# marbl/MHAP

Measured on AMD Instinct MI355X. Metric: overlaps/sec, higher is better.
Workload: dtype int64

## Files before the change

mhap_amd/csrc/kernels.hpp:

```cpp
#pragma once
#include "device_common.hpp"

namespace mhap {

constexpr int HASH_TILE = 1024;
constexpr int WEIGHT_THREADS = 1024;
constexpr int WEIGHT_MAXIT = 24;
constexpr int MH_U = 4;
constexpr int ORD_THREADS = 256;
constexpr int ORD_BINS = 2048;
constexpr int CAND_TQ = 128;
constexpr int CAND_TM = 128;
constexpr int CAND_KS = 32;
constexpr int OVL_THREADS = 128;
#ifndef MH_INV_CT
#define MH_INV_CT 2048
#endif
constexpr int INV_CT = MH_INV_CT;

constexpr int BS_WCLASSES = 6;
constexpr int BS_WMAX = 32;
struct StrandInfo { int32_t valid; int32_t mode; int32_t cnt[BS_WCLASSES + 1]; int32_t pad; };

struct FilterTable {
// ... 22 lines not shown
};

void launch_hash_kmers(hipStream_t st, const ReadDesc* descs, int64_t nstrands, int max_len, const uint8_t* store, int64_t* keys,
                       int32_t* h32, int k, int k2, const uint64_t* luts, int only_mat);
void build_kmer_hash_luts(uint64_t* out);
int weight_grid(int num_cus, int64_t nstrands, int max_len, int k);
bool strand_hashes_from_codes(int length, int k, int k2);
void launch_kmer_weights(hipStream_t st, int num_cus, const ReadDesc* descs, int64_t nstrands, int max_len, const int64_t* keys,
                         uint32_t* wts, uint32_t* perm, uint32_t* slabs, int64_t slab_entries, unsigned long long* counter, int k,
                         const FilterTable& ft, double repeat_weight, StrandInfo* info, bool fused, const uint8_t* store,
                         const uint64_t* luts, const int32_t* order, int32_t* slist);
bool launch_minhash(hipStream_t st, hipStream_t st_weighted, int nblocks, int64_t n_unweighted, int64_t n_weighted, const ReadDesc* descs, int64_t nstrands, const int64_t* keys, const uint32_t* wts,
                    const uint32_t* perm, const StrandInfo* info, const uint8_t* store, const uint64_t* luts, int k, int k2, int H,
                    unsigned long long* counter, int32_t* out_rows, int64_t out_stride, int32_t* out_status, int64_t status_stride,
                    const uint64_t* jump, int jump_na, const int32_t* slist, uint32_t* qbuf, const uint64_t* unjump, const uint64_t* jump_w1, unsigned long long* merge,
                    int max_nk);
size_t minhash_merge_bytes(int nblocks, int H);
void build_xorshift_unjump_tables(int na, int nq, uint64_t* out);
int minhash_wgs_per_cu(int H);
size_t minhash_queue_bytes(int nblocks_total, int H);
int minhash_queue_words(int H);
constexpr int XS_JUMP_LOG2 = 2;
constexpr int XS_JUMP_NQ = BS_WMAX;
#ifndef MH_W1_JUMP_NA
#define MH_W1_JUMP_NA 16
#endif
constexpr int W1_JUMP_NA = MH_W1_JUMP_NA;
inline int w1_jump_tables(int H) { return W1_JUMP_NA + ((H + 1) >> XS_JUMP_LOG2) / W1_JUMP_NA + 1; }
void build_xorshift_jump_tables(int na, int nq, uint64_t* out);
void launch_fix_status(hipStream_t st, int32_t* meta, int64_t nreads);
size_t ordered_lds_bytes(int cap, int code_words, int stage_wide);
void launch_ordered(hipStream_t st, const ReadDesc* descs, int64_t nstrands, int max_len_codes, int max_len, const int32_t* h32,
                    const uint8_t* store, const uint64_t* luts, int k2, int S, int cap, int32_t* out_rows, int64_t out_stride,
                    int32_t* out_meta, int64_t meta_stride, int64_t first = 0, int64_t count = -1);

void launch_candidates(hipStream_t st, const int32_t* minhash, int64_t row_stride, const int32_t* qminhash, int64_t qrow_stride,
                       const int32_t* qlist, int nq, int ne, const int64_t* ids, const int64_t* qids, const int32_t* meta,
                       const int32_t* qmeta, const SearchParams& sp, const long long* rowstart, long long nblocks_tri, Candidate* cand,
                       unsigned long long* cand_count, unsigned long long cand_cap);
constexpr int MHAP_MAX_NUM_HASHES = 8192;
int minhash_waves_per_workgroup(int H);
struct InvIndex {
  uint32_t* ends;
  uint2* items;
  uint32_t nb, shift;
  uint64_t slot_stride;
  uint32_t ne;
  uint32_t grouped;
  uint32_t group_t, class_log;
  uint32_t* lines;
  uint32_t nl_log, line_lb, line_ebits;
  uint32_t tile_entries, tiles;
  uint2* staged;
  uint32_t* tile_counts;
  uint32_t* bin_start;
  uint32_t* bin_long;
};
void launch_query_iota(hipStream_t st, int32_t* qlist, int first, int n);
int index_tile_entries(int ne);
void index_group_params(int64_t entries, InvIndex& ix);
int index_coarse_bins();
bool index_line_params(int64_t entries, uint32_t nb, uint32_t& nl_log, uint32_t& lb, uint32_t& ebits);
size_t index_line_bytes(int H, uint32_t nl_log);
int index_max_buckets_log();
void launch_index_verify(hipStream_t st, const int32_t* minhash, int64_t row_stride, const int32_t* meta, int ne, int H, const InvIndex& ix,
                         unsigned long long* missing);
bool launch_index_build(hipStream_t st, const int32_t* minhash, int64_t row_stride, const int32_t* meta, int ne, int H, const InvIndex& ix);
// ... 33 lines not shown
```

mhap_amd/csrc/mhap_capi.hip:

```cpp
#include <algorithm>
#include <atomic>
#include <cmath>
#include <cstdio>
#include <cstdlib>
#include <chrono>
#include <cstring>
#include <condition_variable>
#include <functional>
#include <mutex>
#include <string>
#include <thread>
#include <vector>

#include "../../include/mhap_hip.h"
static double hp_now() { return std::chrono::duration<double, std::milli>(std::chrono::steady_clock::now().time_since_epoch()).count(); }
#define HPROF(tag) do { if (getenv("MHAP_HOST_PROF")) fprintf(stderr, "[host] %-28s %.3f ms\n", tag, hp_now()); } while (0)
#define DBGSYNC(h, tag) do { if (getenv("MHAP_DEBUG_SYNC")) { fprintf(stderr, "[dbg] %s launched\n", tag); hipError_t _e = hipStreamSynchronize((h)->stream); fprintf(stderr, "[dbg] %s done: %s\n", tag, hipGetErrorString(_e)); } } while (0)
#include "kernels.hpp"
#include "mhap_internal.hpp"
#include "overlap_lane.hpp"

using namespace mhap;

namespace {
// ... 420 lines not shown
    unsigned long long* ctr = h->counters.as<unsigned long long>();
    const ReadDesc* dd = h->descs.as<ReadDesc>();
    HIPCHK(h, hipMemcpyAsync(h->descs.p, h->h_descs, (size_t)nb * sizeof(ReadDesc), hipMemcpyHostToDevice, h->stream));
    HIPCHK(h, hipMemsetAsync(h->counters.p, 0, 256, h->stream));
    const bool fused = k == 16 && k2 == 12;
    if (any_mat) {
      time_begin(h, MHAP_K_HASH);
      launch_hash_kmers(h->stream, dd, nstr, B.max_len, h->store.as<uint8_t>(), h->keys.as<int64_t>(), h->h32.as<int32_t>(), k, k2,
                        h->hash_luts.as<uint64_t>(), 1);
      time_end(h);
      DBGSYNC(h, "hash_kmers");
    }
    HPROF("sketch: descriptors up");
    time_begin(h, MHAP_K_WEIGHT);
    launch_kmer_weights(h->stream, h->num_cus, dd, nstr, B.max_len, h->keys.as<int64_t>(), h->wts.as<uint32_t>(), h->perm.as<uint32_t>(),
                        h->slabs.as<uint32_t>(), slab_entries, ctr + 0, k, h->ft, h->P.repeat_weight, h->info.as<StrandInfo>(), fused,
                        h->store.as<uint8_t>(), h->hash_luts.as<uint64_t>(), d_order, h->slist.as<int32_t>());
    time_end(h);
    DBGSYNC(h, "kmer_weights");
    int per_cu = minhash_wgs_per_cu(H);
    if (const char* e = getenv("MHAP_MINHASH_WGS_PER_CU")) { int v = atoi(e); if (v >= 1 && v <= 8) per_cu = v; }
    int mblocks = h->num_cus * per_cu;
    if (eager_x) mblocks = std::max(per_cu, mblocks - dist_eager_reserve_wgs(h));
    HIPCHK(h, h->mhq.ensure(minhash_queue_bytes(2 * std::max(mblocks, 1), H) * (size_t)(minhash_waves_per_workgroup(H) < 4 ? 4 : 1)));
    HIPCHK(h, h->mhmerge.ensure(minhash_merge_bytes(std::max(mblocks, 1), H)));
    unsigned long long lens[2] = {0, 0};
    HIPCHK(h, hipMemcpyAsync(lens, ctr + 4, 16, hipMemcpyDeviceToHost, h->stream));
    { const int rs = sync_stream(h); if (rs != MHAP_OK) return rs; }
    HPROF("sketch: list lengths back");
    const hipStream_t ost = h->stream;
    auto do_ordered = [&](int64_t first, int64_t count) -> int {
      time_begin(h, MHAP_K_ORDERED, ost);
      launch_ordered(ost, dd, nstr, max_len_codes, B.max_len, h->h32.as<int32_t>(), h->store.as<uint8_t>(), h->hash_luts.as<uint64_t>(), k2, S, h->ord_cap,
                     ord_rows, ord_stride, meta_rows, META_W, first, count);
      time_end(h, ost);
      return MHAP_OK;
    };
    const int ord_first_env = []() { const char* e = getenv("MHAP_ORDERED_FIRST"); return e ? atoi(e) : 0; }();
    const int ord_split_env = []() { const char* e = getenv("MHAP_ORDERED_SPLIT"); const int v = e ? atoi(e) : -1; return v > 100 ? 100 : v; }();
    int64_t batch_read_bases = 0;
    for (int64_t i = 0; i < nb; i++) batch_read_bases += h->h_descs[(size_t)i].length;
    const bool split_pays = batch_read_bases >= 900000000LL && (int64_t)lens[0] >= 4 * (int64_t)lens[1];
    int64_t ord_pre = ord_first_env ? nstr : (nstr * (int64_t)(ord_split_env >= 0 ? ord_split_env : (split_pays ? 55 : 0))) / 100;
    ord_pre &= ~(int64_t)1;
    bool ordered_done = false;
    if (ord_pre > 0 && !eager_x) {
      (void)do_ordered(0, ord_pre);
      ordered_done = ord_pre >= nstr;
      const int nowait = []() { const char* e = getenv("MHAP_ORDERED_NOWAIT"); return e ? atoi(e) : 1; }();
      if (!nowait) {
        HIPCHK(h, hipEventRecord(h->ev_mh_fork, h->stream));
        HIPCHK(h, hipStreamWaitEvent(h->mh_stream, h->ev_mh_fork, 0));
      }
    } else ord_pre = 0;
    if (eager_x) {
      (void)do_ordered(0, nstr);
      ordered_done = true;
      const int rxo = dist_eager_ordered(h, h->stream, ord_rows);
      if (rxo != MHAP_OK) return rxo;
    }
    {
      const int prefill = []() { const char* e = getenv("MHAP_W1_PREFILL"); return e ? atoi(e) : 0; }();
      if (ord_first_env == 2) (void)hipStreamSynchronize(h->stream);
      for (int i = 0; i < prefill; i++) (void)hipMemsetAsync(h->mhq.p, 0, h->mhq.cap, h->stream);
    }
    const size_t t_mh = time_begin(h, MHAP_K_MINHASH);
    const bool mh_forked = launch_minhash(h->stream, h->mh_stream, mblocks, (int64_t)lens[0], (int64_t)lens[1], dd, nstr, h->keys.as<int64_t>(), h->wts.as<uint32_t>(),
// ... 1221 lines not shown
```

mhap_amd/csrc/sketch_kernels.hip:

```cpp
#include <cstdlib>
#include <cstring>

#include "kernels.hpp"
#include <algorithm>
#ifdef MH_ORD_PATHS
#include <cstdio>
#include <string>
#include <vector>
#endif

namespace mhap {

constexpr int HASH_SEG = 4096;
constexpr int HASH_LUT_WORDS = 3 * 256;

void build_kmer_hash_luts(uint64_t* out) {
  const uint64_t c1 = 0x87c37b91114253d5ULL, c2 = 0x4cf5ad432745937fULL;
  const uint32_t d1 = 0xcc9e2d51U, d2 = 0x1b873593U;
  const char* acgt = "ACGT";
  for (int idx = 0; idx < 256; idx++) {
    uint64_t block = 0;
    for (int c = 0; c < 4; c++) block |= (uint64_t)(uint8_t)acgt[(idx >> (2 * c)) & 3] << (16 * c);
    uint64_t k1 = block * c1; k1 = rotl64(k1, 31); k1 *= c2;
    uint64_t k2 = block * c2; k2 = rotl64(k2, 33); k2 *= c1;
    uint32_t a = (uint32_t)block, b = (uint32_t)(block >> 32);
    a *= d1; a = rotl32(a, 15); a *= d2;
    b *= d1; b = rotl32(b, 15); b *= d2;
    out[idx] = k1; out[256 + idx] = k2; out[512 + idx] = (uint64_t)a | ((uint64_t)b << 32);
  }
}

__device__ __forceinline__ uint32_t strand_codes16(const uint8_t* __restrict__ pk, int L, int rcs, int i0) {
  const uint32_t* W = (const uint32_t*)pk;
  const int nd = (((L + 3) >> 2) + 3) >> 2;
  int f0 = rcs ? (L - 16 - i0) : i0;
  if (f0 <= -16 || f0 >= 16 * nd) return 0u;
  int sh = 0;
  if (f0 < 0) { sh = -2 * f0; f0 = 0; }
  const int d = f0 >> 4;
  const uint32_t d0 = W[d], d1 = W[d + 1 < nd ? d + 1 : nd - 1];
  uint32_t x = __builtin_amdgcn_alignbit(d1, d0, (uint32_t)(2 * (f0 & 15))) << sh;
  if (rcs) {
    x = __builtin_bswap32(x);
    x = ((x >> 4) & 0x0f0f0f0fu) | ((x & 0x0f0f0f0fu) << 4);
    x = ((x >> 2) & 0x33333333u) | ((x & 0x33333333u) << 2);
    x = ~x;
  }
  return x;
}

__device__ __forceinline__ uint32_t codes_at(const uint32_t* codes, int p) {
  return __builtin_amdgcn_alignbit(codes[(p >> 4) + 1], codes[p >> 4], (uint32_t)(2 * (p & 15)));
}
__device__ __forceinline__ uint32_t strand_window16(const uint32_t* __restrict__ W, int nd, int L, int rcs, int p) {
  int f0 = rcs ? (L - 16 - p) : p;
  int sh = 0;
  if (f0 < 0) { sh = -2 * f0; f0 = 0; }
  const int i0 = f0 >> 4;
  const uint32_t d0 = W[i0 < nd ? i0 : nd - 1], d1 = W[i0 + 1 < nd ? i0 + 1 : nd - 1];
  uint32_t x = __builtin_amdgcn_alignbit(d1, d0, (uint32_t)(2 * (f0 & 15))) << sh;
  if (rcs) {
    x = __builtin_bswap32(x);
    x = ((x >> 4) & 0x0f0f0f0fu) | ((x & 0x0f0f0f0fu) << 4);
    x = ((x >> 2) & 0x33333333u) | ((x & 0x33333333u) << 2);
    x = ~x;
  }
  return x;
}
__device__ __forceinline__ uint64_t mul5(uint64_t x) {
  uint64_t r;
  asm("v_lshl_add_u64 %0, %1, 2, %1" : "=v"(r) : "v"(x));
  return r;
}
// ... 1765 lines not shown
        float pms = 0.f; (void)hipEventElapsedTime(&pms, pe0, pe1);
        fprintf(stderr, "[minhash w1 prof] launch %.3f ms, %d waves: mean shader clock %.0f MHz (wave-clocks / waves / time)\n", pms, nb * 4,
                pms > 0.f ? tot / ((double)nb * 4.0) / ((double)pms * 1e3) : 0.0);
        fprintf(stderr, "[minhash w1 prof] rows %llu (first-type %llu)  wave-clocks: total %.3g  key load+transpose %.1f%%  first-row slots %.1f%% (%.0f clocks/step)  "
                        "later-row slots %.1f%% (%.0f clocks/step)  drains %.1f%%  candidates/row %.0f\n", hp[4], hp[5], tot, 100.0 * hp[0] / tot, 100.0 * hp[1] / tot,
                hp[5] ? (double)hp[1] / ((double)hp[5] * H) : 0.0, 100.0 * hp[2] / tot, hp[4] > hp[5] ? (double)hp[2] / ((double)(hp[4] - hp[5]) * H) : 0.0,
                100.0 * hp[3] / tot, hp[4] ? (double)hp[6] / (double)hp[4] : 0.0);
      } else
        if (qcap == BS_QCAP) hipLaunchKernelGGL((minhash_w1_kernel<false, true>), dim3(nb), dim3(256), lds1, st, a);
        else hipLaunchKernelGGL((minhash_w1_kernel<false, false>), dim3(nb), dim3(256), lds1, st, a);
      if (a.n_tail > 0)
        hipLaunchKernelGGL(minhash_w1_finish_kernel, dim3((unsigned)((a.n_tail * (long long)H + 255) / 256)), dim3(256), 0, st, a);
      if (witness) snprintf(w1_path, sizeof(w1_path), "w1 n_whole %lld n_tail %lld rmax %d stagger %d", (long long)a.n_whole, (long long)a.n_tail, a.rmax, a.stagger);
    }
    if (witness)
      fprintf(stderr, "[minhash] strands %lld weight-1 %lld weighted %lld nblocks %d: weight-1 launch %s; weighted launch %s\n", (long long)nstrands,
              (long long)n_unweighted, (long long)n_weighted, nblocks, w1_path, nb_w > 0 ? (split ? "split" : "wave") : "none");
    return nb_w > 0;
  }
}


#ifdef MH_ORD_PROF
__device__ unsigned long long g_ord_prof[8];
#define ORD_TICK(k) do { __syncthreads(); if (threadIdx.x == 0) { const unsigned long long t_ = wall_clock64(); atomicAdd(&g_ord_prof[k], t_ - ord_t0); ord_t0 = t_; } } while (0)
#else
#define ORD_TICK(k) do { } while (0)
#endif
#ifdef MH_ORD_PATHS
__device__ uint32_t* g_ord_paths;
#define ORD_PATH_VARS uint32_t ord_att = 0; int ord_lv = 0
#define ORD_PATH_ATT(a) do { ord_att = (uint32_t)(a); } while (0)
#define ORD_PATH_LEVEL(l) do { ord_lv = (l); } while (0)
#define ORD_PATH_HOW(how) do { if (threadIdx.x == 0 && g_ord_paths) g_ord_paths[blockIdx.x] = ord_att | ((uint32_t)(how) << 4) | (stage_wide ? 256u : 0u) | (mat ? 512u : 0u); } while (0)
#define ORD_PATH_NETWORK ORD_PATH_HOW(n > cap ? 4 + ord_lv : 1)
#else
#define ORD_PATH_VARS do { } while (0)
#define ORD_PATH_ATT(a) do { } while (0)
#define ORD_PATH_LEVEL(l) do { } while (0)
#define ORD_PATH_HOW(how) do { } while (0)
#define ORD_PATH_NETWORK do { } while (0)
#endif
__device__ __forceinline__ uint32_t mm3_mul5c(uint32_t h) {
  uint32_t t;
  asm("v_lshl_add_u32 %0, %1, 2, %1" : "=v"(t) : "v"(h));
  return t + 0xe6546b64U;
}
constexpr uint32_t ORD_BUCKET_MAX = 32;
__device__ inline uint64_t okey(int32_t h, int pos) { return ((uint64_t)((uint32_t)h ^ 0x80000000u) << 32) | (uint32_t)pos; }

__global__ __launch_bounds__(ORD_THREADS) void ordered_kernel(const ReadDesc* __restrict__ descs, int64_t nstrands,
                                                              const int32_t* __restrict__ h32, const uint8_t* __restrict__ store,
                                                              const uint64_t* __restrict__ luts, int code_words, int stage_wide, int k2, int S, int cap,
                                                              int32_t* __restrict__ out_rows, int64_t out_stride,
                                                              int32_t* __restrict__ out_meta, int64_t meta_stride, int64_t first) {
  extern __shared__ __attribute__((aligned(16))) char smem[];
  uint32_t* hist = (uint32_t*)smem;
  uint32_t* part = hist + ORD_BINS;
  uint32_t* svars = part + ORD_THREADS;
  uint64_t* buf = (uint64_t*)(svars + 4);
  uint16_t* bstart = (uint16_t*)(buf + cap);
  uint32_t* stage = (uint32_t*)(bstart + ORD_BINS + 2);
  uint16_t* stage16 = (uint16_t*)stage;
  const size_t lut_off = ((size_t)ORD_BINS * 4 + (size_t)ORD_THREADS * 4 + 16 + (size_t)cap * 8 + (size_t)(ORD_BINS + 2) * 2 + (size_t)cap * (stage_wide ? 4 : 2) + 7) & ~(size_t)7;
  uint64_t* lut = (uint64_t*)(smem + lut_off);
  uint32_t* codes = (uint32_t*)(lut + 256);
  uint32_t& s_bin = svars[0]; uint32_t& s_below = svars[1]; uint32_t& s_cnt = svars[2]; uint32_t& s_fill = svars[3];
  const int64_t strand = first + (int64_t)blockIdx.x;
  if (strand >= nstrands) return;
#ifdef MH_ORD_PROF
  unsigned long long ord_t0 = wall_clock64();
#endif
  const ReadDesc rd = descs[strand >> 1];
  const int rcs = (int)(strand & 1);
  const int n = rd.length - k2 + 1;
  int32_t* meta = out_meta + strand * meta_stride;
  if (strand_skipped(rd, rcs) || n < 1) {
    if (threadIdx.x == 0) { meta[0] = 0; meta[1] = n; meta[2] = rd.length; }
    return;
  }
  const bool mat = (rd.flags & MHAP_RD_MAT) != 0;
  const int32_t* hp = h32 + rd.h2_off + (rcs ? rd.h2_stride : 0);
  if (!mat) {
    for (int i = threadIdx.x; i < 256; i += ORD_THREADS) lut[i] = luts[512 + i];
    const int ncw = (rd.length + 15) / 16 + 2;
    for (int wj = threadIdx.x; wj < ncw && wj < code_words; wj += ORD_THREADS) codes[wj] = strand_codes16(store + rd.base_off, rd.length, rcs, 16 * wj);
    __syncthreads();
  }
  ORD_TICK(0);
  auto hget = [&](int i) -> int32_t {
    if (mat) return hp[i];
    const uint32_t cw = codes_at(codes, i);
    uint32_t h = 0;
#pragma unroll
    for (int q = 0; q < 3; q++) {
      const uint64_t kk = lut[(cw >> (8 * q)) & 255u];
      h ^= (uint32_t)kk;         h = rotl32(h, 13); h = mm3_mul5c(h);
      h ^= (uint32_t)(kk >> 32); h = rotl32(h, 13); h = mm3_mul5c(h);
    }
    h ^= 24u;
    return (int32_t)fmix32(h);
  };
  const int K = S < n ? S : n;
  if (threadIdx.x == 0) { meta[0] = K; meta[1] = n; meta[2] = rd.length; }
  if (K <= 0) return;
  ORD_PATH_VARS;

  const double ksig = sqrt((double)K), csig = sqrt((double)cap);
  const double target = fmin((double)K + 7.0 * ksig, (double)cap - 5.0 * csig);
  if (n > cap && target >= (double)K + 3.0 * ksig) {
    const double quant = target / (double)n;
    const uint32_t cut_u = quant >= 1.0 ? 0xFFFFFFFFu : (uint32_t)(quant * 4294967296.0);
    const uint32_t cutbin = cut_u >> 21;
    for (uint32_t j = threadIdx.x; j < ORD_BINS; j += ORD_THREADS) hist[j] = 0;
    if (threadIdx.x == 0) { s_fill = 0; s_cnt = 0; }
    __syncthreads();
    const int lane = threadIdx.x & 63;
    for (int ib = 0; ib < n; ib += 8 * ORD_THREADS) {
      const int p0 = ib + 32 * (int)(threadIdx.x >> 2) + (int)(threadIdx.x & 3);
      int32_t hv[8];
      if (mat) {
#pragma unroll
        for (int u = 0; u < 8; u++) { const int i = p0 + 4 * u; hv[u] = i < n ? hp[i] : 0; }
      } else if (p0 < n) {
        const int d = p0 >> 4;
        const uint32_t sh = (uint32_t)(2 * (p0 & 15));
        const uint32_t w0 = codes[d], w1 = codes[d + 1], w2 = codes[d + 2], w3 = codes[d + 3];
        const uint32_t a[3] = {__builtin_amdgcn_alignbit(w1, w0, sh), __builtin_amdgcn_alignbit(w2, w1, sh), __builtin_amdgcn_alignbit(w3, w2, sh)};
        uint64_t g[10];
#pragma unroll
        for (int j = 0; j < 10; j++) g[j] = lut[(a[j >> 2] >> (8 * (j & 3))) & 255u];
#pragma unroll
        for (int u = 0; u < 8; u++) {
          uint32_t h = 0;
#pragma unroll
          for (int q = 0; q < 3; q++) {
            const uint64_t kk = g[u + q];
            h ^= (uint32_t)kk;         h = rotl32(h, 13); h = mm3_mul5c(h);
            h ^= (uint32_t)(kk >> 32); h = rotl32(h, 13); h = mm3_mul5c(h);
          }
          h ^= 24u;
          hv[u] = (int32_t)fmix32(h);
        }
      } else {
#pragma unroll
        for (int u = 0; u < 8; u++) hv[u] = 0;
      }
      unsigned long long bal[8];
      uint32_t total = 0;
#pragma unroll
      for (int u = 0; u < 8; u++) {
        bal[u] = __ballot(p0 + 4 * u < n && ((uint32_t)hv[u] ^ 0x80000000u) < cut_u);
        total += (uint32_t)__popcll(bal[u]);
      }
      if (total) {
        uint32_t base = 0;
        if (lane == 0) base = atomicAdd(&s_fill, total);
        base = (uint32_t)__builtin_amdgcn_readfirstlane((int)base);
#pragma unroll
        for (int u = 0; u < 8; u++) {
          if ((bal[u] >> lane) & 1ULL) {
            const uint32_t idx = base + __builtin_amdgcn_mbcnt_hi((uint32_t)(bal[u] >> 32), __builtin_amdgcn_mbcnt_lo((uint32_t)bal[u], 0u));
            if (idx < (uint32_t)cap) { if (stage_wide) stage[idx] = (uint32_t)(p0 + 4 * u); else stage16[idx] = (uint16_t)(p0 + 4 * u); }
            atomicAdd(&hist[((uint32_t)hv[u] ^ 0x80000000u) >> 21], 1u);
          }
          base += (uint32_t)__popcll(bal[u]);
        }
      }
    }
    __syncthreads();
    ORD_TICK(1);
    const uint32_t m = s_fill;
    bool ok = m >= (uint32_t)K && m <= (uint32_t)cap;
    ORD_PATH_ATT(m < (uint32_t)K ? 2 : m > (uint32_t)cap ? 3 : 1);
    if (ok) {
      const int per = ORD_BINS / ORD_THREADS;
      uint32_t loc = 0, mx = 0;
      for (int j = 0; j < per; j++) { const uint32_t c = hist[threadIdx.x * per + j]; loc += c; mx = c > mx ? c : mx; }
      uint32_t incl = loc;
#pragma unroll
      for (int off = 1; off < 64; off <<= 1) { const uint32_t v = __shfl_up(incl, off); if (lane >= off) incl += v; }
      if (lane == 63) part[threadIdx.x >> 6] = incl;
      if (mx > ORD_BUCKET_MAX) atomicMax(&s_cnt, mx);
      __syncthreads();
      for (unsigned w = 0; w < (threadIdx.x >> 6); w++) incl += part[w];
      uint32_t run = incl - loc;
      for (int j = 0; j < per; j++) { const uint32_t b = threadIdx.x * per + j; bstart[b] = (uint16_t)run; run += hist[b]; }
      ok = s_cnt == 0;
      __syncthreads();
      if (!ok) ORD_PATH_ATT(4);
    }
    ORD_TICK(2);
    if (ok) {
      for (uint32_t b = threadIdx.x; b <= cutbin; b += ORD_THREADS) hist[b] = 0;
      __syncthreads();
      for (uint32_t t0 = threadIdx.x; t0 < m; t0 += 4 * ORD_THREADS) {
        int ii[4]; uint64_t key[4]; uint32_t slot[4];
#pragma unroll
        for (int u = 0; u < 4; u++) { const uint32_t t = t0 + (uint32_t)u * ORD_THREADS; ii[u] = t < m ? (stage_wide ? (int)stage[t] : (int)stage16[t]) : 0; }
#pragma unroll
        for (int u = 0; u < 4; u++) key[u] = okey(hget(ii[u]), ii[u]);
#pragma unroll
        for (int u = 0; u < 4; u++) { const uint32_t b = (uint32_t)(key[u] >> 53); slot[u] = t0 + (uint32_t)u * ORD_THREADS < m ? (uint32_t)bstart[b] + atomicAdd(&hist[b], 1u) : 0xFFFFFFFFu; }
#pragma unroll
        for (int u = 0; u < 4; u++) if (slot[u] != 0xFFFFFFFFu) buf[slot[u]] = key[u];
      }
      __syncthreads();
      ORD_TICK(3);
      int32_t* orow = out_rows + strand * out_stride;
      for (uint32_t t0 = threadIdx.x; t0 < m; t0 += 2 * ORD_THREADS) {
        uint64_t key[2]; uint32_t s0[2], c[2], rank[2] = {0u, 0u};
#pragma unroll
        for (int u = 0; u < 2; u++) {
          const uint32_t t = t0 + (uint32_t)u * ORD_THREADS;
          key[u] = buf[t < m ? t : t0];
          const uint32_t b = (uint32_t)(key[u] >> 53);
          s0[u] = bstart[b]; c[u] = t < m ? hist[b] : 0u;
        }
        const uint32_t cmax = c[0] > c[1] ? c[0] : c[1];
        for (uint32_t q = 0; q < cmax; q += 4) {
          uint64_t o[2][4];
#pragma unroll
          for (int u = 0; u < 2; u++)
#pragma unroll
            for (int x = 0; x < 4; x++) o[u][x] = buf[s0[u] + q + (uint32_t)x < (uint32_t)cap ? s0[u] + q + (uint32_t)x : s0[u]];
#pragma unroll
          for (int u = 0; u < 2; u++)
#pragma unroll
            for (int x = 0; x < 4; x++) rank[u] += (q + (uint32_t)x < c[u] && o[u][x] < key[u]) ? 1u : 0u;
        }
#pragma unroll
        for (int u = 0; u < 2; u++) {
          const uint32_t j = s0[u] + rank[u];
          if (t0 + (uint32_t)u * ORD_THREADS < m && j < (uint32_t)K) { orow[2 * j] = (int32_t)((uint32_t)(key[u] >> 32) ^ 0x80000000u); orow[2 * j + 1] = (int32_t)(uint32_t)key[u]; }
        }
      }
      ORD_TICK(5);
#ifdef MH_ORD_PROF
      if (threadIdx.x == 0) atomicAdd(&g_ord_prof[7], 1ULL);
#endif
      ORD_PATH_HOW(2);
      return;
    }
    __syncthreads();
  }

  uint64_t bound = ~0ULL;
  bool buckets = false;
  uint32_t bk_bin = 0, bk_total = 0;
  if (threadIdx.x == 0) s_fill = 0;
  if (n > cap) {
    const int shifts[6] = {53, 42, 32, 21, 10, 0};
    const int widths[6] = {11, 11, 10, 11, 11, 10};
    uint64_t prefix = 0;
    uint64_t prefmask = 0;
    uint32_t below = 0;
    for (int lv = 0; lv < 6; lv++) {
      const int sh = shifts[lv];
      const uint32_t nb = 1u << widths[lv];
      for (uint32_t j = threadIdx.x; j < ORD_BINS; j += ORD_THREADS) hist[j] = 0;
      __syncthreads();
      for (int i0 = threadIdx.x; i0 < n; i0 += 8 * ORD_THREADS) {
        int32_t hv[8];
#pragma unroll
        for (int u = 0; u < 8; u++) { const int i = i0 + u * ORD_THREADS; hv[u] = i < n ? hget(i) : 0; }
#pragma unroll
        for (int u = 0; u < 8; u++) {
// ... 86 lines not shown
    ORD_PATH_HOW(3);
    return;
  }
  ORD_PATH_NETWORK;
  __syncthreads();
  for (int i = threadIdx.x; i < n; i += ORD_THREADS) {
    const uint64_t key = okey(hget(i), i);
    if (key <= bound) { uint32_t slot = atomicAdd(&s_fill, 1u); if (slot < (uint32_t)cap) buf[slot] = key; }
  }
  __syncthreads();
  const uint32_t m = s_fill < (uint32_t)cap ? s_fill : (uint32_t)cap;
  uint32_t np2 = 1;
  while (np2 < m) np2 <<= 1;
  for (uint32_t j = m + threadIdx.x; j < np2; j += ORD_THREADS) buf[j] = ~0ULL;
  __syncthreads();
  for (uint32_t size = 2; size <= np2; size <<= 1) {
    for (uint32_t stride = size >> 1; stride > 0; stride >>= 1) {
      for (uint32_t t = threadIdx.x; t < (np2 >> 1); t += ORD_THREADS) {
        const uint32_t lo = 2 * t - (t & (stride - 1));
        const uint32_t hi = lo + stride;
        const bool up = ((lo & size) == 0);
        const uint64_t a = buf[lo], b = buf[hi];
        if ((a > b) == up) { buf[lo] = b; buf[hi] = a; }
      }
      __syncthreads();
    }
  }
  int32_t* orow = out_rows + strand * out_stride;
  for (int j = threadIdx.x; j < K; j += ORD_THREADS) {
    const uint64_t key = buf[j];
    orow[2 * j] = (int32_t)((uint32_t)(key >> 32) ^ 0x80000000u);
    orow[2 * j + 1] = (int32_t)(uint32_t)key;
  }
}

#ifndef MH_ORD_PAD
#define MH_ORD_PAD 0
#endif
size_t ordered_lds_bytes(int cap, int code_words, int stage_wide) {
  return (size_t)ORD_BINS * 4 + (size_t)ORD_THREADS * 4 + 16 + (size_t)cap * 8 + (size_t)(ORD_BINS + 2) * 2 + (size_t)cap * (stage_wide ? 4 : 2) +
         (code_words > 0 ? (size_t)256 * 8 + (size_t)code_words * 4 : 0) + 8 + MH_ORD_PAD;
}

__global__ void fix_status_kernel(int32_t* __restrict__ meta, int64_t nreads) {
  const int64_t i = (int64_t)blockIdx.x * blockDim.x + threadIdx.x;
  if (i >= nreads) return;
  const int32_t fs = meta[(2 * i) * META_W + 3];
  if (fs != 0 && meta[(2 * i + 1) * META_W + 3] == 0) meta[(2 * i + 1) * META_W + 3] = fs;
}

void launch_fix_status(hipStream_t st, int32_t* meta, int64_t nreads) {
  if (nreads <= 0) return;
  hipLaunchKernelGGL(fix_status_kernel, dim3((unsigned)((nreads + 255) / 256)), dim3(256), 0, st, meta, nreads);
}

void launch_ordered(hipStream_t st, const ReadDesc* descs, int64_t nstrands, int max_len_codes, int max_len, const int32_t* h32,
                    const uint8_t* store, const uint64_t* luts, int k2, int S, int cap, int32_t* out_rows, int64_t out_stride,
                    int32_t* out_meta, int64_t meta_stride, int64_t first, int64_t count) {
  if (count < 0 || first + count > nstrands) count = nstrands - first;
  if (nstrands <= 0 || count <= 0) return;
  const int code_words = max_len_codes > 0 ? (max_len_codes + 15) / 16 + 4 : 0;
  const int stage_wide = max_len - k2 + 1 > 65535 ? 1 : 0;
#ifdef MH_ORD_PATHS
  uint32_t* d_paths = nullptr;
  if (hipMalloc(&d_paths, (size_t)count * sizeof(uint32_t)) != hipSuccess) d_paths = nullptr;
  if (d_paths) (void)hipMemsetAsync(d_paths, 0, (size_t)count * sizeof(uint32_t), st);
  (void)hipStreamSynchronize(st);
  (void)hipMemcpyToSymbol(HIP_SYMBOL(g_ord_paths), &d_paths, sizeof(d_paths));
#endif
  hipLaunchKernelGGL(ordered_kernel, dim3((unsigned)count), dim3(ORD_THREADS), ordered_lds_bytes(cap, code_words, stage_wide), st, descs, nstrands, h32,
                     store, luts, code_words, stage_wide, k2, S, cap, out_rows, out_stride, out_meta, meta_stride, first);
#ifdef MH_ORD_PROF
  (void)hipStreamSynchronize(st);
  unsigned long long hp[8];
  (void)hipMemcpyFromSymbol(hp, HIP_SYMBOL(g_ord_prof), sizeof(hp));
  fprintf(stderr, "[ordered prof] cap %d lds %zu strands(one-pass) %llu  100MHz ticks/strand: stage %.1f pass1 %.1f scan %.1f fill %.1f isort %.1f out %.1f\n", cap,
          ordered_lds_bytes(cap, code_words, stage_wide), hp[7], (double)hp[0] / hp[7], (double)hp[1] / hp[7], (double)hp[2] / hp[7], (double)hp[3] / hp[7],
          (double)hp[4] / hp[7], (double)hp[5] / hp[7]);
  unsigned long long z[8] = {0, 0, 0, 0, 0, 0, 0, 0};
  (void)hipMemcpyToSymbol(HIP_SYMBOL(g_ord_prof), z, sizeof(z));
#endif
#ifdef MH_ORD_PATHS
  {
    std::vector<uint32_t> h_paths((size_t)count, 0u);
    if (d_paths) (void)hipMemcpyAsync(h_paths.data(), d_paths, (size_t)count * sizeof(uint32_t), hipMemcpyDeviceToHost, st);
    (void)hipStreamSynchronize(st);
    if (d_paths) (void)hipFree(d_paths);
    std::string line;
    line.reserve((size_t)count * 4 + 96);
    char tmp[96];
    snprintf(tmp, sizeof(tmp), "[ordered paths] first %lld count %lld cap %d S %d codes:", (long long)first, (long long)count, cap, S);
    line += tmp;
    for (uint32_t c : h_paths) { snprintf(tmp, sizeof(tmp), " %03x", c & 0xFFFu); line += tmp; }
    fprintf(stderr, "%s\n", line.c_str());
  }
#endif
}

}
```

Measured before the change: 451,600.

## Make ordered kernel persistent with prefetch, single-pass key staging and finer bins

```diff
diff --git a/mhap_amd/csrc/kernels.hpp b/mhap_amd/csrc/kernels.hpp
--- a/mhap_amd/csrc/kernels.hpp
+++ b/mhap_amd/csrc/kernels.hpp
@@ -78,7 +78,7 @@
 size_t ordered_lds_bytes(int cap, int code_words, int stage_wide);
 void launch_ordered(hipStream_t st, const ReadDesc* descs, int64_t nstrands, int max_len_codes, int max_len, const int32_t* h32,
                     const uint8_t* store, const uint64_t* luts, int k2, int S, int cap, int32_t* out_rows, int64_t out_stride,
-                    int32_t* out_meta, int64_t meta_stride, int64_t first = 0, int64_t count = -1);
+                    int32_t* out_meta, int64_t meta_stride, int num_cus, int64_t first = 0, int64_t count = -1);
 
 void launch_candidates(hipStream_t st, const int32_t* minhash, int64_t row_stride, const int32_t* qminhash, int64_t qrow_stride,
                        const int32_t* qlist, int nq, int ne, const int64_t* ids, const int64_t* qids, const int32_t* meta,
diff --git a/mhap_amd/csrc/mhap_capi.hip b/mhap_amd/csrc/mhap_capi.hip
--- a/mhap_amd/csrc/mhap_capi.hip
+++ b/mhap_amd/csrc/mhap_capi.hip
@@ -476,7 +476,7 @@
     auto do_ordered = [&](int64_t first, int64_t count) -> int {
       time_begin(h, MHAP_K_ORDERED, ost);
       launch_ordered(ost, dd, nstr, max_len_codes, B.max_len, h->h32.as<int32_t>(), h->store.as<uint8_t>(), h->hash_luts.as<uint64_t>(), k2, S, h->ord_cap,
-                     ord_rows, ord_stride, meta_rows, META_W, first, count);
+                     ord_rows, ord_stride, meta_rows, META_W, h->num_cus, first, count);
       time_end(h, ost);
       return MHAP_OK;
     };
diff --git a/mhap_amd/csrc/sketch_kernels.hip b/mhap_amd/csrc/sketch_kernels.hip
--- a/mhap_amd/csrc/sketch_kernels.hip
+++ b/mhap_amd/csrc/sketch_kernels.hip
@@ -39,6 +39,32 @@
   if (f0 < 0) { sh = -2 * f0; f0 = 0; }
   const int d = f0 >> 4;
   const uint32_t d0 = W[d], d1 = W[d + 1 < nd ? d + 1 : nd - 1];
+  uint32_t x = __builtin_amdgcn_alignbit(d1, d0, (uint32_t)(2 * (f0 & 15))) << sh;
+  if (rcs) {
+    x = __builtin_bswap32(x);
+    x = ((x >> 4) & 0x0f0f0f0fu) | ((x & 0x0f0f0f0fu) << 4);
+    x = ((x >> 2) & 0x33333333u) | ((x & 0x33333333u) << 2);
+    x = ~x;
+  }
+  return x;
+}
+
+__device__ __forceinline__ void codes16_fetch(const uint8_t* __restrict__ pk, int L, int rcs, int i0, uint32_t& d0, uint32_t& d1) {
+  const uint32_t* W = (const uint32_t*)pk;
+  const int nd = (((L + 3) >> 2) + 3) >> 2;
+  int f0 = rcs ? (L - 16 - i0) : i0;
+  d0 = 0u; d1 = 0u;
+  if (f0 <= -16 || f0 >= 16 * nd) return;
+  if (f0 < 0) f0 = 0;
+  const int d = f0 >> 4;
+  d0 = W[d]; d1 = W[d + 1 < nd ? d + 1 : nd - 1];
+}
+__device__ __forceinline__ uint32_t codes16_finish(int L, int rcs, int i0, uint32_t d0, uint32_t d1) {
+  const int nd = (((L + 3) >> 2) + 3) >> 2;
+  int f0 = rcs ? (L - 16 - i0) : i0;
+  if (f0 <= -16 || f0 >= 16 * nd) return 0u;
+  int sh = 0;
+  if (f0 < 0) { sh = -2 * f0; f0 = 0; }
   uint32_t x = __builtin_amdgcn_alignbit(d1, d0, (uint32_t)(2 * (f0 & 15))) << sh;
   if (rcs) {
     x = __builtin_bswap32(x);
@@ -1870,7 +1896,7 @@
 #define ORD_PATH_VARS uint32_t ord_att = 0; int ord_lv = 0
 #define ORD_PATH_ATT(a) do { ord_att = (uint32_t)(a); } while (0)
 #define ORD_PATH_LEVEL(l) do { ord_lv = (l); } while (0)
-#define ORD_PATH_HOW(how) do { if (threadIdx.x == 0 && g_ord_paths) g_ord_paths[blockIdx.x] = ord_att | ((uint32_t)(how) << 4) | (stage_wide ? 256u : 0u) | (mat ? 512u : 0u); } while (0)
+#define ORD_PATH_HOW(how) do { if (threadIdx.x == 0 && g_ord_paths) g_ord_paths[strand - first] = ord_att | ((uint32_t)(how) << 4) | (stage_wide ? 256u : 0u) | (mat ? 512u : 0u); } while (0)
 #define ORD_PATH_NETWORK ORD_PATH_HOW(n > cap ? 4 + ord_lv : 1)
 #else
 #define ORD_PATH_VARS do { } while (0)
@@ -1885,31 +1911,54 @@
   return t + 0xe6546b64U;
 }
 constexpr uint32_t ORD_BUCKET_MAX = 32;
+#ifndef MH_ORD_ONCE_CAP
+#define MH_ORD_ONCE_CAP (8 * ORD_THREADS)
+#endif
+#ifndef MH_ORD_FINE_MAX
+#define MH_ORD_FINE_MAX 3
+#endif
+constexpr int ORD_BUF_PAD = 4;
+constexpr int ORD_ONCE_CAP = MH_ORD_ONCE_CAP;
+static_assert(ORD_ONCE_CAP <= 8 * ORD_THREADS && MH_ORD_FINE_MAX >= 0 && MH_ORD_FINE_MAX <= 3, "eight keys per lane; a lane's slice of eight counters holds whole groups");
 __device__ inline uint64_t okey(int32_t h, int pos) { return ((uint64_t)((uint32_t)h ^ 0x80000000u) << 32) | (uint32_t)pos; }
 
-__global__ __launch_bounds__(ORD_THREADS) void ordered_kernel(const ReadDesc* __restrict__ descs, int64_t nstrands,
+template <bool ONCE>
+__global__ __launch_bounds__(ORD_THREADS) __attribute__((amdgpu_waves_per_eu(4, 8))) void ordered_kernel(const ReadDesc* __restrict__ descs, int64_t nstrands,
                                                               const int32_t* __restrict__ h32, const uint8_t* __restrict__ store,
                                                               const uint64_t* __restrict__ luts, int code_words, int stage_wide, int k2, int S, int cap,
                                                               int32_t* __restrict__ out_rows, int64_t out_stride,
-                                                              int32_t* __restrict__ out_meta, int64_t meta_stride, int64_t first) {
+                                                              int32_t* __restrict__ out_meta, int64_t meta_stride, int64_t first, int64_t count) {
   extern __shared__ __attribute__((aligned(16))) char smem[];
   uint32_t* hist = (uint32_t*)smem;
   uint32_t* part = hist + ORD_BINS;
   uint32_t* svars = part + ORD_THREADS;
   uint64_t* buf = (uint64_t*)(svars + 4);
-  uint16_t* bstart = (uint16_t*)(buf + cap);
+  uint16_t* bstart = (uint16_t*)(buf + cap + ORD_BUF_PAD);
   uint32_t* stage = (uint32_t*)(bstart + ORD_BINS + 2);
   uint16_t* stage16 = (uint16_t*)stage;
-  const size_t lut_off = ((size_t)ORD_BINS * 4 + (size_t)ORD_THREADS * 4 + 16 + (size_t)cap * 8 + (size_t)(ORD_BINS + 2) * 2 + (size_t)cap * (stage_wide ? 4 : 2) + 7) & ~(size_t)7;
+  const size_t lut_off = ((size_t)ORD_BINS * 4 + (size_t)ORD_THREADS * 4 + 16 + (size_t)(cap + ORD_BUF_PAD) * 8 + (size_t)(ORD_BINS + 2) * 2 + (ONCE ? (size_t)0 : (size_t)cap * (stage_wide ? 4 : 2)) + 7) & ~(size_t)7;
   uint64_t* lut = (uint64_t*)(smem + lut_off);
   uint32_t* codes = (uint32_t*)(lut + 256);
   uint32_t& s_bin = svars[0]; uint32_t& s_below = svars[1]; uint32_t& s_cnt = svars[2]; uint32_t& s_fill = svars[3];
-  const int64_t strand = first + (int64_t)blockIdx.x;
-  if (strand >= nstrands) return;
+  static_assert(ORD_THREADS == 256, "one table entry per lane");
+  if (code_words > 0) lut[threadIdx.x] = luts[512 + threadIdx.x];
+  auto wants_codes = [&](int64_t i, const ReadDesc& d) {
+    return i < count && !(d.flags & MHAP_RD_MAT) && !strand_skipped(d, (int)((first + i) & 1)) && d.length - k2 + 1 >= 1;
+  };
+  auto load_codes = [&](int64_t i, const ReadDesc& d, uint32_t (&w)[8]) {
+    const int ncw = (d.length + 15) / 16 + 2;
+    const int lim = ncw < code_words ? ncw : code_words;
+#pragma unroll
+    for (int u = 0; u < 4; u++) {
+      const int wj = threadIdx.x + u * ORD_THREADS;
+      w[2 * u] = 0u; w[2 * u + 1] = 0u;
+      if (wj < lim) codes16_fetch(store + d.base_off, d.length, (int)((first + i) & 1), 16 * wj, w[2 * u], w[2 * u + 1]);
+    }
+  };
+  auto run = [&](const int64_t strand, const ReadDesc& rd, const uint32_t (&pcw)[8]) {
 #ifdef MH_ORD_PROF
   unsigned long long ord_t0 = wall_clock64();
 #endif
-  const ReadDesc rd = descs[strand >> 1];
   const int rcs = (int)(strand & 1);
   const int n = rd.length - k2 + 1;
   int32_t* meta = out_meta + strand * meta_stride;
@@ -1920,9 +1969,11 @@
   const bool mat = (rd.flags & MHAP_RD_MAT) != 0;
   const int32_t* hp = h32 + rd.h2_off + (rcs ? rd.h2_stride : 0);
   if (!mat) {
-    for (int i = threadIdx.x; i < 256; i += ORD_THREADS) lut[i] = luts[512 + i];
     const int ncw = (rd.length + 15) / 16 + 2;
-    for (int wj = threadIdx.x; wj < ncw && wj < code_words; wj += ORD_THREADS) codes[wj] = strand_codes16(store + rd.base_off, rd.length, rcs, 16 * wj);
+    const int lim = ncw < code_words ? ncw : code_words;
+#pragma unroll
+    for (int u = 0; u < 4; u++) { const int wj = threadIdx.x + u * ORD_THREADS; if (wj < lim) codes[wj] = codes16_finish(rd.length, rcs, 16 * wj, pcw[2 * u], pcw[2 * u + 1]); }
+    for (int wj = threadIdx.x + 4 * ORD_THREADS; wj < lim; wj += ORD_THREADS) codes[wj] = strand_codes16(store + rd.base_off, rd.length, rcs, 16 * wj);
     __syncthreads();
   }
   ORD_TICK(0);
@@ -1950,6 +2001,10 @@
     const double quant = target / (double)n;
     const uint32_t cut_u = quant >= 1.0 ? 0xFFFFFFFFu : (uint32_t)(quant * 4294967296.0);
     const uint32_t cutbin = cut_u >> 21;
+    int f = 0;
+    while (f < MH_ORD_FINE_MAX && ((cutbin + 1) << (f + 1)) <= (uint32_t)ORD_BINS) f++;
+    const uint32_t nfb = (cutbin + 1) << f;
+    const int hsh = 21 - f, ksh = 53 - f;
     for (uint32_t j = threadIdx.x; j < ORD_BINS; j += ORD_THREADS) hist[j] = 0;
     if (threadIdx.x == 0) { s_fill = 0; s_cnt = 0; }
     __syncthreads();
@@ -1999,8 +2054,12 @@
         for (int u = 0; u < 8; u++) {
           if ((bal[u] >> lane) & 1ULL) {
             const uint32_t idx = base + __builtin_amdgcn_mbcnt_hi((uint32_t)(bal[u] >> 32), __builtin_amdgcn_mbcnt_lo((uint32_t)bal[u], 0u));
-            if (idx < (uint32_t)cap) { if (stage_wide) stage[idx] = (uint32_t)(p0 + 4 * u); else stage16[idx] = (uint16_t)(p0 + 4 * u); }
-            atomicAdd(&hist[((uint32_t)hv[u] ^ 0x80000000u) >> 21], 1u);
+            if (idx < (uint32_t)cap) {
+              if (ONCE) buf[idx] = okey(hv[u], p0 + 4 * u);
+              else if (stage_wide) stage[idx] = (uint32_t)(p0 + 4 * u);
+              else stage16[idx] = (uint16_t)(p0 + 4 * u);
+            }
+            atomicAdd(&hist[((uint32_t)hv[u] ^ 0x80000000u) >> hsh], 1u);
           }
           base += (uint32_t)__popcll(bal[u]);
         }
@@ -2012,9 +2071,15 @@
     bool ok = m >= (uint32_t)K && m <= (uint32_t)cap;
     ORD_PATH_ATT(m < (uint32_t)K ? 2 : m > (uint32_t)cap ? 3 : 1);
     if (ok) {
-      const int per = ORD_BINS / ORD_THREADS;
-      uint32_t loc = 0, mx = 0;
-      for (int j = 0; j < per; j++) { const uint32_t c = hist[threadIdx.x * per + j]; loc += c; mx = c > mx ? c : mx; }
+      const uint4 ca = ((const uint4*)hist)[2 * threadIdx.x], cb = ((const uint4*)hist)[2 * threadIdx.x + 1];
+      const uint32_t c8[8] = {ca.x, ca.y, ca.z, ca.w, cb.x, cb.y, cb.z, cb.w};
+      const uint32_t gmask = (1u << f) - 1u;
+      uint32_t loc = 0, mx = 0, acc = 0;
+#pragma unroll
+      for (int j = 0; j < 8; j++) {
+        loc += c8[j]; acc += c8[j];
+        if ((((uint32_t)j + 1u) & gmask) == 0u) { mx = acc > mx ? acc : mx; acc = 0; }
+      }
       uint32_t incl = loc;
 #pragma unroll
       for (int off = 1; off < 64; off <<= 1) { const uint32_t v = __shfl_up(incl, off); if (lane >= off) incl += v; }
@@ -2023,54 +2088,115 @@
       __syncthreads();
       for (unsigned w = 0; w < (threadIdx.x >> 6); w++) incl += part[w];
       uint32_t run = incl - loc;
-      for (int j = 0; j < per; j++) { const uint32_t b = threadIdx.x * per + j; bstart[b] = (uint16_t)run; run += hist[b]; }
+      uint32_t* bs32 = (uint32_t*)bstart + 4 * threadIdx.x;
+#pragma unroll
+      for (int j = 0; j < 4; j++) {
+        const uint32_t lo = run; run += c8[2 * j];
+        const uint32_t hi = run; run += c8[2 * j + 1];
+        bs32[j] = (lo & 0xFFFFu) | (hi << 16);
+      }
       ok = s_cnt == 0;
       __syncthreads();
       if (!ok) ORD_PATH_ATT(4);
     }
     ORD_TICK(2);
     if (ok) {
-      for (uint32_t b = threadIdx.x; b <= cutbin; b += ORD_THREADS) hist[b] = 0;
-      __syncthreads();
-      for (uint32_t t0 = threadIdx.x; t0 < m; t0 += 4 * ORD_THREADS) {
-        int ii[4]; uint64_t key[4]; uint32_t slot[4];
-#pragma unroll
-        for (int u = 0; u < 4; u++) { const uint32_t t = t0 + (uint32_t)u * ORD_THREADS; ii[u] = t < m ? (stage_wide ? (int)stage[t] : (int)stage16[t]) : 0; }
-#pragma unroll
-        for (int u = 0; u < 4; u++) key[u] = okey(hget(ii[u]), ii[u]);
-#pragma unroll
-        for (int u = 0; u < 4; u++) { const uint32_t b = (uint32_t)(key[u] >> 53); slot[u] = t0 + (uint32_t)u * ORD_THREADS < m ? (uint32_t)bstart[b] + atomicAdd(&hist[b], 1u) : 0xFFFFFFFFu; }
-#pragma unroll
-        for (int u = 0; u < 4; u++) if (slot[u] != 0xFFFFFFFFu) buf[slot[u]] = key[u];
-      }
-      __syncthreads();
-      ORD_TICK(3);
       int32_t* orow = out_rows + strand * out_stride;
-      for (uint32_t t0 = threadIdx.x; t0 < m; t0 += 2 * ORD_THREADS) {
-        uint64_t key[2]; uint32_t s0[2], c[2], rank[2] = {0u, 0u};
-#pragma unroll
-        for (int u = 0; u < 2; u++) {
-          const uint32_t t = t0 + (uint32_t)u * ORD_THREADS;
-          key[u] = buf[t < m ? t : t0];
-          const uint32_t b = (uint32_t)(key[u] >> 53);
-          s0[u] = bstart[b]; c[u] = t < m ? hist[b] : 0u;
+      const bool row8 = (((uintptr_t)orow) & 7u) == 0;
+      auto put = [&](uint32_t j, uint64_t key) {
+        const int32_t hh = (int32_t)((uint32_t)(key >> 32) ^ 0x80000000u), pp = (int32_t)(uint32_t)key;
+        if (row8) *(int2*)(orow + 2 * (size_t)j) = make_int2(hh, pp);
+        else { orow[2 * (size_t)j] = hh; orow[2 * (size_t)j + 1] = pp; }
+      };
+      if (ONCE) {
+        static_assert(ORD_BINS == 8 * ORD_THREADS, "a lane's slice of the histogram is eight counters; ONCE holds cap / ORD_THREADS <= 8 keys per lane");
+        uint64_t key[8]; uint32_t s0[8], slot[8];
+#pragma unroll
+        for (int u = 0; u < 8; u++) { const uint32_t t = threadIdx.x + (uint32_t)u * ORD_THREADS; key[u] = t < m ? buf[t] : ~0ULL; }
+        for (uint32_t b = threadIdx.x; b < nfb; b += ORD_THREADS) hist[b] = 0;
+        __syncthreads();
+#pragma unroll
+        for (int u = 0; u < 8; u++) {
+          const bool live = threadIdx.x + (uint32_t)u * ORD_THREADS < m;
+          const uint32_t b = live ? (uint32_t)(key[u] >> ksh) : 0u;
+          s0[u] = live ? (uint32_t)bstart[b] : 0u;
+          slot[u] = live ? s0[u] + atomicAdd(&hist[b], 1u) : 0xFFFFFFFFu;
         }
-        const uint32_t cmax = c[0] > c[1] ? c[0] : c[1];
-        for (uint32_t q = 0; q < cmax; q += 4) {
-          uint64_t o[2][4];
-#pragma unroll
-          for (int u = 0; u < 2; u++)
-#pragma unroll
-            for (int x = 0; x < 4; x++) o[u][x] = buf[s0[u] + q + (uint32_t)x < (uint32_t)cap ? s0[u] + q + (uint32_t)x : s0[u]];
-#pragma unroll
-          for (int u = 0; u < 2; u++)
-#pragma unroll
-            for (int x = 0; x < 4; x++) rank[u] += (q + (uint32_t)x < c[u] && o[u][x] < key[u]) ? 1u : 0u;
+#pragma unroll
+        for (int u = 0; u < 8; u++) if (slot[u] < (uint32_t)cap) buf[slot[u]] = key[u];
+        __syncthreads();
+        ORD_TICK(3);
+#pragma unroll
+        for (int hb = 0; hb < 8; hb += 4) {
+          if ((uint32_t)hb * ORD_THREADS >= m) break;
+          uint32_t c[4], rank[4] = {0u, 0u, 0u, 0u}, cmax = 0;
+#pragma unroll
+          for (int u = 0; u < 4; u++) {
+            const bool live = threadIdx.x + (uint32_t)(hb + u) * ORD_THREADS < m;
+            c[u] = live ? hist[(uint32_t)(key[hb + u] >> ksh)] : 0u;
+            cmax = c[u] > cmax ? c[u] : cmax;
+          }
+          for (uint32_t q = 0; q < cmax; q += 4) {
+            uint64_t o[4][4];
+#pragma unroll
+            for (int u = 0; u < 4; u++) {
+              const uint64_t* src = buf + s0[hb + u] + (q < c[u] ? q : 0u);
+#pragma unroll
+              for (int x = 0; x < 4; x++) o[u][x] = src[x];
+            }
+#pragma unroll
+            for (int u = 0; u < 4; u++)
+#pragma unroll
+              for (int x = 0; x < 4; x++) rank[u] += (q + (uint32_t)x < c[u] && o[u][x] < key[hb + u]) ? 1u : 0u;
+          }
+#pragma unroll
+          for (int u = 0; u < 4; u++) {
+            const uint32_t j = s0[hb + u] + rank[u];
+            if (c[u] != 0u && j < (uint32_t)K) put(j, key[hb + u]);
+          }
         }
-#pragma unroll
-        for (int u = 0; u < 2; u++) {
-          const uint32_t j = s0[u] + rank[u];
-          if (t0 + (uint32_t)u * ORD_THREADS < m && j < (uint32_t)K) { orow[2 * j] = (int32_t)((uint32_t)(key[u] >> 32) ^ 0x80000000u); orow[2 * j + 1] = (int32_t)(uint32_t)key[u]; }
+      } else {
+        for (uint32_t b = threadIdx.x; b < nfb; b += ORD_THREADS) hist[b] = 0;
+        __syncthreads();
+        for (uint32_t t0 = threadIdx.x; t0 < m; t0 += 4 * ORD_THREADS) {
+          int ii[4]; uint64_t key[4]; uint32_t slot[4];
+#pragma unroll
+          for (int u = 0; u < 4; u++) { const uint32_t t = t0 + (uint32_t)u * ORD_THREADS; ii[u] = t < m ? (stage_wide ? (int)stage[t] : (int)stage16[t]) : 0; }
+#pragma unroll
+          for (int u = 0; u < 4; u++) key[u] = okey(hget(ii[u]), ii[u]);
+#pragma unroll
+          for (int u = 0; u < 4; u++) { const uint32_t b = (uint32_t)(key[u] >> ksh); slot[u] = t0 + (uint32_t)u * ORD_THREADS < m ? (uint32_t)bstart[b] + atomicAdd(&hist[b], 1u) : 0xFFFFFFFFu; }
+#pragma unroll
+          for (int u = 0; u < 4; u++) if (slot[u] != 0xFFFFFFFFu) buf[slot[u]] = key[u];
+        }
+        __syncthreads();
+        ORD_TICK(3);
+        for (uint32_t t0 = threadIdx.x; t0 < m; t0 += 2 * ORD_THREADS) {
+          uint64_t key[2]; uint32_t s0[2], c[2], rank[2] = {0u, 0u};
+#pragma unroll
+          for (int u = 0; u < 2; u++) {
+            const uint32_t t = t0 + (uint32_t)u * ORD_THREADS;
+            key[u] = buf[t < m ? t : t0];
+            const uint32_t b = (uint32_t)(key[u] >> ksh);
+            s0[u] = bstart[b]; c[u] = t < m ? hist[b] : 0u;
+          }
+          const uint32_t cmax = c[0] > c[1] ? c[0] : c[1];
+          for (uint32_t q = 0; q < cmax; q += 4) {
+            uint64_t o[2][4];
+#pragma unroll
+            for (int u = 0; u < 2; u++)
+#pragma unroll
+              for (int x = 0; x < 4; x++) o[u][x] = buf[s0[u] + q + (uint32_t)x < (uint32_t)cap ? s0[u] + q + (uint32_t)x : s0[u]];
+#pragma unroll
+            for (int u = 0; u < 2; u++)
+#pragma unroll
+              for (int x = 0; x < 4; x++) rank[u] += (q + (uint32_t)x < c[u] && o[u][x] < key[u]) ? 1u : 0u;
+          }
+#pragma unroll
+          for (int u = 0; u < 2; u++) {
+            const uint32_t j = s0[u] + rank[u];
+            if (t0 + (uint32_t)u * ORD_THREADS < m && j < (uint32_t)K) put(j, key[u]);
+          }
         }
       }
       ORD_TICK(5);
@@ -2223,13 +2349,33 @@
     orow[2 * j] = (int32_t)((uint32_t)(key >> 32) ^ 0x80000000u);
     orow[2 * j + 1] = (int32_t)(uint32_t)key;
   }
+  };
+
+  const int64_t step = (int64_t)gridDim.x;
+  int64_t i = (int64_t)blockIdx.x;
+  ReadDesc rd = {}, nrd = {};
+  uint32_t cw[8] = {0u, 0u, 0u, 0u, 0u, 0u, 0u, 0u};
+  if (i < count) rd = descs[(first + i) >> 1];
+  if (i + step < count) nrd = descs[(first + i + step) >> 1];
+  if (wants_codes(i, rd)) load_codes(i, rd, cw);
+  for (; i < count; i += step) {
+    ReadDesc nnrd = {};
+    if (i + 2 * step < count) nnrd = descs[(first + i + 2 * step) >> 1];
+    uint32_t ncw[8] = {0u, 0u, 0u, 0u, 0u, 0u, 0u, 0u};
+    if (wants_codes(i + step, nrd)) load_codes(i + step, nrd, ncw);
+    run(first + i, rd, cw);
+    __syncthreads();
+    rd = nrd; nrd = nnrd;
+#pragma unroll
+    for (int u = 0; u < 8; u++) cw[u] = ncw[u];
+  }
 }
 
 #ifndef MH_ORD_PAD
 #define MH_ORD_PAD 0
 #endif
 size_t ordered_lds_bytes(int cap, int code_words, int stage_wide) {
-  return (size_t)ORD_BINS * 4 + (size_t)ORD_THREADS * 4 + 16 + (size_t)cap * 8 + (size_t)(ORD_BINS + 2) * 2 + (size_t)cap * (stage_wide ? 4 : 2) +
+  return (size_t)ORD_BINS * 4 + (size_t)ORD_THREADS * 4 + 16 + (size_t)(cap + ORD_BUF_PAD) * 8 + (size_t)(ORD_BINS + 2) * 2 + (cap <= ORD_ONCE_CAP ? (size_t)0 : (size_t)cap * (stage_wide ? 4 : 2)) +
          (code_words > 0 ? (size_t)256 * 8 + (size_t)code_words * 4 : 0) + 8 + MH_ORD_PAD;
 }
 
@@ -2247,7 +2393,7 @@
 
 void launch_ordered(hipStream_t st, const ReadDesc* descs, int64_t nstrands, int max_len_codes, int max_len, const int32_t* h32,
                     const uint8_t* store, const uint64_t* luts, int k2, int S, int cap, int32_t* out_rows, int64_t out_stride,
-                    int32_t* out_meta, int64_t meta_stride, int64_t first, int64_t count) {
+                    int32_t* out_meta, int64_t meta_stride, int num_cus, int64_t first, int64_t count) {
   if (count < 0 || first + count > nstrands) count = nstrands - first;
   if (nstrands <= 0 || count <= 0) return;
   const int code_words = max_len_codes > 0 ? (max_len_codes + 15) / 16 + 4 : 0;
@@ -2259,15 +2405,20 @@
   (void)hipStreamSynchronize(st);
   (void)hipMemcpyToSymbol(HIP_SYMBOL(g_ord_paths), &d_paths, sizeof(d_paths));
 #endif
-  hipLaunchKernelGGL(ordered_kernel, dim3((unsigned)count), dim3(ORD_THREADS), ordered_lds_bytes(cap, code_words, stage_wide), st, descs, nstrands, h32,
-                     store, luts, code_words, stage_wide, k2, S, cap, out_rows, out_stride, out_meta, meta_stride, first);
+  const auto kern = cap <= ORD_ONCE_CAP ? ordered_kernel<true> : ordered_kernel<false>;
+  const size_t lds = ordered_lds_bytes(cap, code_words, stage_wide);
+  int per_cu = 0;
+  if (hipOccupancyMaxActiveBlocksPerMultiprocessor(&per_cu, kern, ORD_THREADS, lds) != hipSuccess || per_cu < 1) per_cu = 1;
+  const int64_t grid = std::min<int64_t>(count, (int64_t)std::max(1, num_cus) * per_cu);
+  hipLaunchKernelGGL(kern, dim3((unsigned)grid), dim3(ORD_THREADS), lds, st, descs, nstrands, h32, store, luts, code_words, stage_wide, k2, S, cap, out_rows,
+                     out_stride, out_meta, meta_stride, first, count);
 #ifdef MH_ORD_PROF
   (void)hipStreamSynchronize(st);
   unsigned long long hp[8];
   (void)hipMemcpyFromSymbol(hp, HIP_SYMBOL(g_ord_prof), sizeof(hp));
-  fprintf(stderr, "[ordered prof] cap %d lds %zu strands(one-pass) %llu  100MHz ticks/strand: stage %.1f pass1 %.1f scan %.1f fill %.1f isort %.1f out %.1f\n", cap,
+  fprintf(stderr, "[ordered prof] cap %d lds %zu strands(one-pass) %llu  100MHz ticks/strand: stage %.1f hash %.1f scan %.1f fill %.1f rank %.1f\n", cap,
           ordered_lds_bytes(cap, code_words, stage_wide), hp[7], (double)hp[0] / hp[7], (double)hp[1] / hp[7], (double)hp[2] / hp[7], (double)hp[3] / hp[7],
-          (double)hp[4] / hp[7], (double)hp[5] / hp[7]);
+          (double)hp[5] / hp[7]);
   unsigned long long z[8] = {0, 0, 0, 0, 0, 0, 0, 0};
   (void)hipMemcpyToSymbol(HIP_SYMBOL(g_ord_prof), z, sizeof(z));
 #endif
```

Result: no change. 453,100, median of 4 (+0.3%).
